# luo-yining/CFDBench

Hardware: NVIDIA H100
Metric: fno_rollout_steps_per_sec (higher is better)
Workload: dtype bf16

## Files before the change

cfdbench_b200/_lib.py:

```python
from __future__ import annotations

import ctypes as C
import os

_HERE = os.path.dirname(os.path.abspath(__file__))
LIB_PATH = os.path.join(_HERE, "libcfdbench_b200.so")

FNO_MAX_LAYERS = 8
ABI_VERSION = 4
ACT_F32, ACT_BF16 = 0, 1
EPI_GELU, EPI_GELU_SAVE_PRE, EPI_MUL_DGELU, EPI_PLAIN = 0, 1, 2, 3


class FnoWeights(C.Structure):
    _fields_ = [
        ("n_layers", C.c_int32),
        ("n_case_params", C.c_int32),
        ("fc0_w", C.c_void_p),
        ("fc0_b", C.c_void_p),
        ("spec_wk", C.c_void_p * FNO_MAX_LAYERS),
        ("w0t", C.c_void_p * FNO_MAX_LAYERS),
        ("w0_b", C.c_void_p * FNO_MAX_LAYERS),
        ("fc1_w", C.c_void_p),
        ("fc1_b", C.c_void_p),
# ... 64 lines not shown
    "fno_bwd_partials_bytes": (C.c_size_t, []),
    "fno_mode_mix_image": (C.c_int, [_P, _P, _P, _I, _P]),
    "fno_block_fused": (C.c_int, [_P, _P, _P, _P, _P, _I, _P]),
    "fno_pack_spectral_weights": (C.c_int, [_P, _P, _P, _I, _P]),
    "fno_unpack_spectral_grads": (C.c_int, [_P, _P, _P, _P]),
    "fno_mix_operand_bytes": (C.c_size_t, []),
    "fno_pack_mix_operand": (C.c_int, [_P, _P, _P]),
    "fno_pack_mix_operand_from_weights": (C.c_int, [_P, _P, _P, _I, _P]),
    "fno_lift_fwd": (C.c_int, [_P, _P, _P, C.POINTER(FnoWeights), _P, _I, _I, _P]),
    "fno_spectral_dft_fwd": (C.c_int, [_P, _P, _I, _I, _F, _F, _P]),
    "fno_mode_mix": (C.c_int, [_P, _P, _P, _I, _P]),
    "fno_spectral_inv_kx": (C.c_int, [_P, _P, _I, _F, _F, _P]),
    "fno_block_out": (C.c_int, [_I, _P, _P, _P, _P, _P, _P, _P, _I, _I, _P]),
    "fno_block_fwd": (C.c_int, [C.POINTER(FnoWeights), _I, _P, _P, _P, C.POINTER(FnoWorkspace), _I, _I, _P]),
    "fno_project_fwd": (C.c_int, [_P, _P, C.POINTER(FnoWeights), _P, _I, _I, _P]),
    "fno_forward": (C.c_int, [C.POINTER(FnoWeights), _P, _P, _P, _P, C.POINTER(FnoWorkspace), _I, _I, _P]),
    "fno_rollout": (C.c_int, [C.POINTER(FnoWeights), _P, _P, _P, _P, _I, C.POINTER(FnoWorkspace), _I, _I, _P]),
    "fno_rollout_host": (C.c_int, [C.POINTER(FnoWeights), _P, _P, _P, _P, _I, C.POINTER(FnoWorkspace), _P, _I, _I, _P]),
    "fno_rollout_host_scratch_bytes": (C.c_size_t, [_I, _I, _I]),
    "fno_multistep_metrics": (C.c_int, [_P, _P, _P, _P, _I, _I, _P]),
    "fno_gather_batch": (C.c_int, [_P, _P, _P, _P, _P, _I, _I, _I, _P, _P, _P, _P, _P]),
    "fno_loss_scratch_bytes": (C.c_size_t, []),
    "fno_loss_fwd": (C.c_int, [_P, _P, C.c_size_t, _P, _P, _P]),
    "fno_loss_bwd": (C.c_int, [_P, _P, _P, _P, _P, C.c_size_t, _P]),
    "fno_adam_step": (C.c_int, [C.POINTER(FnoAdamTensors), C.c_float, C.c_float, C.c_float, C.c_float, C.c_float,
                                C.c_int64, _P]),
    "fno_train_stage_indices": (C.c_int, [_P, C.c_int64, _I, _I, _P, _P, _P]),
    "fno_adam_step_dev": (C.c_int, [C.POINTER(FnoAdamTensors), _P, _I, _P, _F, _F, _F, _F, _P]),
    "fno_adam_coefficients": (C.c_int, [_F, _F, _F, C.c_int64, _I, _P]),
    "fno_train_log_step": (C.c_int, [_P, _P, _I, _P, _P]),
# ... 78 lines not shown
```

cfdbench_b200/build.py:

```python
from __future__ import annotations

import hashlib
import os
import subprocess
import sys
import time

HERE = os.path.dirname(os.path.abspath(__file__))
CSRC = os.path.join(HERE, "csrc")
OUT = os.path.join(HERE, "libcfdbench_b200.so")
STAMP = os.path.join(HERE, ".build_stamp")
SOURCES = ["fno_abi.cu", "fno_dft_fwd.cu", "fno_dft_fwd_tc.cu", "fno_mode_mix.cu", "fno_block_tc.cu", "fno_block_fused.cu", "fno_pointwise.cu", "fno_project_tc.cu", "fno_project_bwd_tc.cu",
           "fno_backward.cu", "fno_metrics.cu", "fno_train_step.cu", "fno_grid.cu"]
NVCC_FLAGS = ["-std=c++17", "-O3", "-lineinfo", "-gencode", "arch=compute_90a,code=sm_90a",
              "-Xcompiler", "-fPIC"]


def _nvcc() -> str:
    for cand in (os.environ.get("NVCC"), "/usr/local/cuda/bin/nvcc"):
        if cand and os.path.exists(cand):
            return cand
    return "nvcc"


def _fingerprint() -> str:
    h = hashlib.sha256()
    for root in (CSRC, os.path.join(os.path.dirname(HERE), "include")):
# ... 52 lines not shown
```

cfdbench_b200/csrc/fno_abi.cu:

```cuda
#include <stdio.h>
#include <string.h>

#include "../../include/cfdbench_b200.h"
#include "fno_common.cuh"

namespace fno {
cudaError_t launch_dft_fwd(const void*, void*, int, float, float, cudaStream_t);
cudaError_t launch_mode_mix(const void*, const void*, void*, void*, int, cudaStream_t);
cudaError_t launch_block_fused(const void*, const void*, const float*, const float*, void*, int, cudaStream_t);
size_t ym_image_bytes(int);
cudaError_t launch_pack_spectral(const void*, const void*, void*, int, cudaStream_t);
cudaError_t launch_unpack_spectral(const void*, void*, void*, int, cudaStream_t);
cudaError_t launch_dft_fwd_tc(const void*, void*, int, float, float, cudaStream_t);
cudaError_t launch_pack_mix_operand(const void*, void*, cudaStream_t);
cudaError_t launch_pack_mix_operand_direct(const void*, const void*, void*, int, cudaStream_t);
size_t mix_operand_bytes();
cudaError_t launch_gather_batch(const void*, const void*, const float*, const int*, const long long*, int, int, int, float*,
                                float*, float*, float*, cudaStream_t);
cudaError_t launch_loss_fwd(const float*, const float*, size_t, float*, float*, cudaStream_t);
cudaError_t launch_loss_bwd(const float*, const float*, const float*, const float*, float*, size_t, cudaStream_t);
size_t loss_scratch_bytes();
cudaError_t launch_adam_step(const fno_adam_tensors*, float, float, float, float, float, long long, cudaStream_t);
cudaError_t launch_adam_step_dev(const fno_adam_tensors*, const float*, int, const int*, float, float, float, float,
                                 cudaStream_t);
void adam_coefficients(float, float, float, long long, float*, float*);
cudaError_t launch_stage_indices(const long long*, long long, int, int, const int*, long long*, cudaStream_t);
cudaError_t launch_log_step(const float*, float*, int, int*, cudaStream_t);
cudaError_t launch_inv_kx(const void*, void*, int, float, float, cudaStream_t);
template <typename TAct>
cudaError_t launch_block_tc(int, const void*, const void*, const float*, const float*, void*, float*, const float*, int,
                            cudaStream_t);
template <typename TAct>
cudaError_t launch_lift(const float*, const float*, const float*, const float*, const float*, const float*,
                        const float*, void*, int, int, cudaStream_t);
template <typename TAct>
cudaError_t launch_project_tc(const void*, const float*, const float*, const float*, const float*, const float*,
                              float*, int, cudaStream_t);
int project_bwd_rows_max();
int project_bwd_row();
cudaError_t launch_reduce_partials(const float*, int, int, float*, int, float*, int, float*, int, int, cudaStream_t);
template <typename TAct>
cudaError_t launch_project_bwd_tc(const void*, const float*, const float*, const float*, const float*, const float*, const float*,
                                  float*, float*, float*, int*, int, cudaStream_t);
template <typename TP, typename TQ, int NJ, int NI>
cudaError_t launch_chan_outer(const void*, const void*, float*, int*, int, cudaStream_t);
cudaError_t launch_multistep_metrics(const float*, const float*, const float*, float*, int, int, cudaStream_t);
cudaError_t launch_spectral_wgrad(const void*, const void*, void*, int, cudaStream_t);
cudaError_t launch_lift_bwd(const float*, const float*, const float*, const float*, const float*, const float*,
                            float*, float*, float*, int, int, int, cudaStream_t);
cudaError_t launch_lift_bwd_data(const float*, const float*, float*, float*, const float*, int, int, int, cudaStream_t);
bool grid_ok(int, int);
void grid_tables_release(int);
// ... 186 lines not shown
  if (act_dtype == FNO_ACT_BF16 && ws->ym_img && !pre_out) {
    FNO_TRY(fno_mode_mix_image(ws->xm, w->spec_wk[layer], ws->ym_img, batch, stream));
    return fno_block_fused(ws->ym_img, act_in, w->w0t[layer], w->w0_b[layer], act_out, batch, stream);
  }
  FNO_TRY(fno_mode_mix(ws->xm, w->spec_wk[layer], ws->ym, batch, stream));
  const float inv = 1.f / static_cast<float>(kHW);
  FNO_TRY(fno_spectral_inv_kx(ws->ym, ws->z, batch, inv, 2.f * inv, stream));
  return fno_block_out(pre_out ? FNO_EPI_GELU_SAVE_PRE : FNO_EPI_GELU, ws->z, act_in, w->w0t[layer], w->w0_b[layer],
                       act_out, pre_out, nullptr, batch, act_dtype, stream);
}

int fno_project_fwd(const void* act_in, const float* mask, const fno_weights* w, float* preds, int batch,
                    int act_dtype, void* stream) {
  if (!act_in || !mask || !w || !preds || batch <= 0 || bad_dtype(act_dtype))
    return fail(kErrArg, "fno_project_fwd: bad argument");
  cudaError_t e =
      act_dtype == FNO_ACT_F32
          ? launch_project_tc<float>(act_in, w->fc1_w, w->fc1_b, w->fc2_w, w->fc2_b, mask, preds, batch, S(stream))
          : launch_project_tc<__nv_bfloat16>(act_in, w->fc1_w, w->fc1_b, w->fc2_w, w->fc2_b, mask, preds, batch, S(stream));
  FNO_CUDA(e, "project_kernel");
  return kOk;
}

int fno_forward(const fno_weights* w, const float* inputs, const float* mask, const float* case_params,
                float* preds, const fno_workspace* ws, int batch, int act_dtype, void* stream) {
  if (!w || !ws || !ws->act[0] || !ws->act[1] || !ws->xm) return fail(kErrArg, "fno_forward: bad workspace");
  if (!(act_dtype == FNO_ACT_BF16 && ws->ym_img) && (!ws->ym || !ws->z)) return fail(kErrArg, "fno_forward: bad workspace");
  if (w->n_layers < 1 || w->n_layers > FNO_MAX_LAYERS) return fail(kErrUnsupported, "fno_forward: n_layers out of range");
  FNO_TRY(fno_lift_fwd(inputs, mask, case_params, w, ws->act[0], batch, act_dtype, stream));
  int cur = 0;
  for (int l = 0; l < w->n_layers; ++l) {
    FNO_TRY(fno_block_fwd(w, l, ws->act[cur], ws->act[cur ^ 1], nullptr, ws, batch, act_dtype, stream));
    cur ^= 1;
  }
  return fno_project_fwd(ws->act[cur], mask, w, preds, batch, act_dtype, stream);
}

int fno_rollout(const fno_weights* w, const float* inputs, const float* mask, const float* case_params,
                float* preds_seq, int steps, const fno_workspace* ws, int batch, int act_dtype, void* stream) {
  if (steps < 0 || !preds_seq) return fail(kErrArg, "fno_rollout: bad argument");
  const size_t frame = static_cast<size_t>(batch) * 2 * kHW;
  const float* cur = inputs;
  for (int s = 0; s < steps; ++s) {
    float* nxt = preds_seq + static_cast<size_t>(s) * frame;
    FNO_TRY(fno_forward(w, cur, mask, case_params, nxt, ws, batch, act_dtype, stream));
    cur = nxt;
  }
  return kOk;
}

size_t fno_rollout_host_scratch_bytes(int batch, int n_case_params, int steps) {
  const size_t b = static_cast<size_t>(batch);
  return (b * 2 * kHW + b * kHW + static_cast<size_t>(steps) * b * 2 * kHW) * sizeof(float) +
         ((b * n_case_params * sizeof(float) + 255) / 256) * 256;
}

int fno_rollout_host(const fno_weights* w, const float* inputs_host, const float* mask_host,
                     const float* case_params_host, float* preds_seq_host, int steps, const fno_workspace* ws,
                     void* dev_io, int batch, int act_dtype, void* stream) {
  if (!w || !inputs_host || !mask_host || !preds_seq_host || !dev_io || batch <= 0 || steps <= 0)
    return fail(kErrArg, "fno_rollout_host: bad argument");
// ... 677 lines not shown
```

cfdbench_b200/csrc/fno_project_tc.cu:

```cuda
#include "fno_common.cuh"
#include "tc_common.cuh"

namespace fno {

constexpr int kPtWG = 4;
constexpr int kPtThreads = 128 * kPtWG;
constexpr int kPtM = kW;
constexpr uint32_t kPtLboA = (kPtM / 8) * 128;
constexpr uint32_t kPtLboB = (kProj / 8) * 128;
constexpr int kPtTilesPerSample = kH;
constexpr int kPtReps = kPtM * (kC / 4) / 128;

struct PtSmem {
  alignas(128) float w_hi[kProj * kC];
  alignas(128) float w_lo[kProj * kC];
  alignas(128) float a_hi[kPtWG][kPtM * kC];
  alignas(128) float a_lo[kPtWG][kPtM * kC];
  alignas(16) float4 w2q[kProj / 2];
  alignas(16) float2 b1p[kProj / 2];
};

template <typename TAct>
struct PtRegs {
  TAct v[kPtReps][4];
};

template <typename TAct>
__device__ __forceinline__ void pt_prefetch(PtRegs<TAct>& r, const TAct* __restrict__ a, int tile, int t) {
  const int b = tile / kPtTilesPerSample, p0 = (tile % kPtTilesPerSample) * kPtM;
#pragma unroll
  for (int rep = 0; rep < kPtReps; ++rep) {
    const int task = rep * 128 + t;
    const int m = task & (kPtM - 1), kq = task >> 6;
    const TAct* src = a + (static_cast<size_t>(b) * kC + 4 * kq) * kHW + p0 + m;
#pragma unroll
    for (int c = 0; c < 4; ++c) r.v[rep][c] = __ldg(src + static_cast<size_t>(c) * kHW);
  }
}

__device__ __forceinline__ float pt_to_float(float v) { return v; }
__device__ __forceinline__ float pt_to_float(__nv_bfloat16 v) { return __bfloat162float(v); }

template <typename TAct>
__device__ __forceinline__ void pt_split_store(const PtRegs<TAct>& r, float* a_hi, float* a_lo, int t) {
#pragma unroll
  for (int rep = 0; rep < kPtReps; ++rep) {
    const int task = rep * 128 + t;
    const int m = task & (kPtM - 1), kq = task >> 6;
    float hi[4], lo[4];
#pragma unroll
    for (int c = 0; c < 4; ++c) {
      const float x = pt_to_float(r.v[rep][c]);
      if constexpr (sizeof(TAct) == 4) tc::split_tf32(x, hi[c], lo[c]);
      else hi[c] = x;
    }
    const uint32_t off = tc::kmajor_offset(m, 4 * kq, kPtM) / 4;
    *reinterpret_cast<float4*>(a_hi + off) = make_float4(hi[0], hi[1], hi[2], hi[3]);
    if constexpr (sizeof(TAct) == 4) *reinterpret_cast<float4*>(a_lo + off) = make_float4(lo[0], lo[1], lo[2], lo[3]);
  }
}

template <typename TAct>
__global__ void __launch_bounds__(kPtThreads, 1)
    project_tc_kernel(const TAct* __restrict__ a, const float* __restrict__ w1, const float* __restrict__ b1,
                      const float* __restrict__ w2, const float* __restrict__ b2, const float* __restrict__ mask,
                      float* __restrict__ preds, int n_tiles) {
  constexpr bool kBf16 = sizeof(TAct) == 2;
  extern __shared__ __align__(1024) unsigned char smem_raw[];
  PtSmem& sm = *reinterpret_cast<PtSmem*>(smem_raw);
  const int tid = threadIdx.x, lane = tid & 31;
  const int wg = tc::warp_index_uniform() >> 2, t = tid & 127, wq = (tid >> 5) & 3;

  for (int e = tid; e < kProj * kC; e += kPtThreads) {
    const int j = e / kC, i = e % kC;
    float hi, lo;
    tc::split_tf32(w1[e], hi, lo);
    const uint32_t off = tc::kmajor_offset(j, i, kProj) / 4;
    sm.w_hi[off] = hi;
    sm.w_lo[off] = lo;
  }
  if (tid < kProj / 2) {
    sm.w2q[tid] = make_float4(w2[2 * tid], w2[kProj + 2 * tid], w2[2 * tid + 1], w2[kProj + 2 * tid + 1]);
    sm.b1p[tid] = make_float2(b1[2 * tid], b1[2 * tid + 1]);
  }
  const float b2x = b2[0], b2y = b2[1];
  tc::fence_proxy_async_smem();
  __syncthreads();
  pdl_wait();
  pdl_launch_dependents();

  const int first = blockIdx.x * kPtWG + wg, stride = gridDim.x * kPtWG;
  float* a_hi = sm.a_hi[wg];
  float* a_lo = sm.a_lo[wg];
  PtRegs<TAct> regs;
  if (first < n_tiles) pt_prefetch<TAct>(regs, a, first, t);
  for (int tile = first; tile < n_tiles; tile += stride) {
    pt_split_store<TAct>(regs, a_hi, a_lo, t);
    tc::fence_proxy_async_smem();
    tc::named_barrier(1 + wg, 128);
    if (tile + stride < n_tiles) pt_prefetch<TAct>(regs, a, tile + stride, t);
    float acc[64];
    tc::wg_fence();
    {
      const uint32_t a_s[3] = {tc::smem_addr(a_hi), tc::smem_addr(a_lo), tc::smem_addr(a_hi)};
      const uint32_t b_s[3] = {tc::smem_addr(sm.w_hi), tc::smem_addr(sm.w_hi), tc::smem_addr(sm.w_lo)};
#pragma unroll
      for (int pass = 0; pass < 3; ++pass) {
        if (kBf16 && pass == 1) continue;
#pragma unroll
        for (int ks = 0; ks < kC / 8; ++ks)
          tc::wg_tf32_ss_n128(acc, tc::make_smem_desc(a_s[pass] + ks * 2 * kPtLboA, kPtLboA, 128),
                              tc::make_smem_desc(b_s[pass] + ks * 2 * kPtLboB, kPtLboB, 128), (pass | ks) ? 1u : 0u);
      }
    }
    tc::wg_commit();
    tc::wg_wait<0>();
    tc::wg_fence_acc(acc);
    const int b = tile / kPtTilesPerSample, p0 = (tile % kPtTilesPerSample) * kPtM;
#pragma unroll
    for (int hh = 0; hh < 2; ++hh) {
      float2 out = make_float2(0.f, 0.f);
#pragma unroll
      for (int i0 = 0; i0 < 16; i0 += 8) {
        float2 g[8];
#pragma unroll
        for (int i = 0; i < 8; ++i) {
          const float2 bb = sm.b1p[4 * (i0 + i) + (lane & 3)];
          g[i] = make_float2(acc[4 * (i0 + i) + 2 * hh] + bb.x, acc[4 * (i0 + i) + 2 * hh + 1] + bb.y);
        }
        if constexpr (kBf16) {
          gelu_erf2_deg5_batch<8>(g);
        } else {
#pragma unroll
          for (int i = 0; i < 8; ++i) g[i] = gelu_erf2(g[i]);
        }
#pragma unroll
        for (int i = 0; i < 8; ++i) {
          const float4 wq4 = sm.w2q[4 * (i0 + i) + (lane & 3)];
          out = ffma2(make_float2(g[i].x, g[i].x), make_float2(wq4.x, wq4.y), out);
          out = ffma2(make_float2(g[i].y, g[i].y), make_float2(wq4.z, wq4.w), out);
        }
      }
      out.x += __shfl_xor_sync(0xffffffffu, out.x, 1);
      out.y += __shfl_xor_sync(0xffffffffu, out.y, 1);
      out.x += __shfl_xor_sync(0xffffffffu, out.x, 2);
      out.y += __shfl_xor_sync(0xffffffffu, out.y, 2);
      if ((lane & 3) == 0) {
        const int pix = p0 + 16 * wq + (lane >> 2) + 8 * hh;
        const float mk = __ldg(mask + static_cast<size_t>(b) * kHW + pix);
        preds[(static_cast<size_t>(b) * 2 + 0) * kHW + pix] = (b2x + out.x) * mk;
        preds[(static_cast<size_t>(b) * 2 + 1) * kHW + pix] = (b2y + out.y) * mk;
      }
    }
  }
}

template <typename TAct>
cudaError_t launch_project_tc(const void* a, const float* w1, const float* b1, const float* w2, const float* b2,
                              const float* mask, float* preds, int batch, cudaStream_t stream) {
  auto kern = project_tc_kernel<TAct>;
  constexpr size_t smem = sizeof(PtSmem);
  static PerDeviceLaunch pd;
  int n_sm = 0;
  cudaError_t e0 = per_device_setup(kern, smem, pd, &n_sm);
  if (e0 != cudaSuccess) return e0;
  const int n_tiles = batch * kPtTilesPerSample;
  const int want = (n_tiles + kPtWG - 1) / kPtWG;
  const int grid = want < n_sm ? want : n_sm;
  return launch_chained(kern, dim3(grid), dim3(kPtThreads), smem, stream, static_cast<const TAct*>(a), w1, b1, w2, b2,
                        mask, preds, n_tiles);
}
template cudaError_t launch_project_tc<float>(const void*, const float*, const float*, const float*, const float*,
                                              const float*, float*, int, cudaStream_t);
template cudaError_t launch_project_tc<__nv_bfloat16>(const void*, const float*, const float*, const float*,
                                                      const float*, const float*, float*, int, cudaStream_t);

}
```

cfdbench_b200/csrc/tc_common.cuh:

```cuda
#pragma once
#include <cuda_runtime.h>
#include <stdint.h>

namespace fno {
namespace tc {

__device__ __forceinline__ uint32_t smem_addr(const void* p) {
  return static_cast<uint32_t>(__cvta_generic_to_shared(p));
}

__device__ __forceinline__ int warp_index_uniform() {
  return __shfl_sync(0xffffffffu, static_cast<int>(threadIdx.x >> 5), 0);
}

__device__ __forceinline__ void named_barrier(int id, int count) {
  asm volatile("bar.sync %0, %1;" ::"r"(id), "r"(count) : "memory");
}

__device__ __forceinline__ void fence_proxy_async_smem() {
  asm volatile("fence.proxy.async.shared::cta;" ::: "memory");
}

__device__ __forceinline__ uint64_t make_smem_desc(uint32_t saddr, uint32_t lbo_bytes, uint32_t sbo_bytes) {
  uint64_t d = 0;
// ... 39 lines not shown
  asm volatile(
      "{\n.reg .pred p;\nsetp.ne.b32 p, %38, 0;\n"
      "wgmma.mma_async.sync.aligned.m64n72k16.f32.bf16.bf16 {%0, %1, %2, %3, %4, %5, %6, %7, %8, %9, %10, %11, %12, %13, %14, %15, %16, %17, %18, %19, %20, %21, %22, %23, %24, %25, %26, %27, %28, %29, %30, %31, %32, %33, %34, %35}, %36, %37, p, 1, 1, 0, 0;\n}\n"
      : "+f"(d[0]), "+f"(d[1]), "+f"(d[2]), "+f"(d[3]), "+f"(d[4]), "+f"(d[5]), "+f"(d[6]), "+f"(d[7]), "+f"(d[8]), "+f"(d[9]), "+f"(d[10]), "+f"(d[11]), "+f"(d[12]), "+f"(d[13]), "+f"(d[14]), "+f"(d[15]), "+f"(d[16]), "+f"(d[17]), "+f"(d[18]), "+f"(d[19]), "+f"(d[20]), "+f"(d[21]), "+f"(d[22]), "+f"(d[23]), "+f"(d[24]), "+f"(d[25]), "+f"(d[26]), "+f"(d[27]), "+f"(d[28]), "+f"(d[29]), "+f"(d[30]), "+f"(d[31]), "+f"(d[32]), "+f"(d[33]), "+f"(d[34]), "+f"(d[35])
      : "l"(a), "l"(b), "r"(acc)
      : "memory");
}
__device__ __forceinline__ void wg_bf16_ss_n32_mn_a(float* d, uint64_t a, uint64_t b, uint32_t acc) {
  asm volatile(
      "{\n.reg .pred p;\nsetp.ne.b32 p, %18, 0;\n"
      "wgmma.mma_async.sync.aligned.m64n32k16.f32.bf16.bf16 {%0, %1, %2, %3, %4, %5, %6, %7, %8, %9, %10, %11, %12, %13, %14, %15}, %16, %17, p, 1, 1, 1, 0;\n}\n"
      : "+f"(d[0]), "+f"(d[1]), "+f"(d[2]), "+f"(d[3]), "+f"(d[4]), "+f"(d[5]), "+f"(d[6]), "+f"(d[7]), "+f"(d[8]), "+f"(d[9]), "+f"(d[10]), "+f"(d[11]), "+f"(d[12]), "+f"(d[13]), "+f"(d[14]), "+f"(d[15])
      : "l"(a), "l"(b), "r"(acc)
      : "memory");
}
__device__ __forceinline__ void wg_tf32_rs_n32(float* d, const uint32_t* a, uint64_t b, uint32_t acc) {
  asm volatile(
      "{\n.reg .pred p;\nsetp.ne.b32 p, %21, 0;\n"
      "wgmma.mma_async.sync.aligned.m64n32k8.f32.tf32.tf32 {%0, %1, %2, %3, %4, %5, %6, %7, %8, %9, %10, %11, %12, %13, %14, %15}, {%16, %17, %18, %19}, %20, p, 1, 1;\n}\n"
      : "+f"(d[0]), "+f"(d[1]), "+f"(d[2]), "+f"(d[3]), "+f"(d[4]), "+f"(d[5]), "+f"(d[6]), "+f"(d[7]), "+f"(d[8]), "+f"(d[9]), "+f"(d[10]), "+f"(d[11]), "+f"(d[12]), "+f"(d[13]), "+f"(d[14]), "+f"(d[15])
      : "r"(a[0]), "r"(a[1]), "r"(a[2]), "r"(a[3]), "l"(b), "r"(acc)
      : "memory");
}
__device__ __forceinline__ void wg_tf32_rs_n48(float* d, const uint32_t* a, uint64_t b, uint32_t acc) {
  asm volatile(
      "{\n.reg .pred p;\nsetp.ne.b32 p, %29, 0;\n"
      "wgmma.mma_async.sync.aligned.m64n48k8.f32.tf32.tf32 {%0, %1, %2, %3, %4, %5, %6, %7, %8, %9, %10, %11, %12, %13, %14, %15, %16, %17, %18, %19, %20, %21, %22, %23}, {%24, %25, %26, %27}, %28, p, 1, 1;\n}\n"
      : "+f"(d[0]), "+f"(d[1]), "+f"(d[2]), "+f"(d[3]), "+f"(d[4]), "+f"(d[5]), "+f"(d[6]), "+f"(d[7]), "+f"(d[8]), "+f"(d[9]), "+f"(d[10]), "+f"(d[11]), "+f"(d[12]), "+f"(d[13]), "+f"(d[14]), "+f"(d[15]), "+f"(d[16]), "+f"(d[17]), "+f"(d[18]), "+f"(d[19]), "+f"(d[20]), "+f"(d[21]), "+f"(d[22]), "+f"(d[23])
      : "r"(a[0]), "r"(a[1]), "r"(a[2]), "r"(a[3]), "l"(b), "r"(acc)
      : "memory");
// ... 24 lines not shown
```

include/cfdbench_b200.h:

```cpp
#ifndef CFDBENCH_B200_H_
#define CFDBENCH_B200_H_

#include <stddef.h>
#include <stdint.h>

#ifdef __cplusplus
extern "C" {
#endif

#define FNO_ABI_VERSION 4
#define FNO_MAX_LAYERS 8

enum { FNO_ACT_F32 = 0, FNO_ACT_BF16 = 1 };
enum { FNO_EPI_GELU = 0, FNO_EPI_GELU_SAVE_PRE = 1, FNO_EPI_MUL_DGELU = 2, FNO_EPI_PLAIN = 3 };

typedef struct fno_weights {
  int32_t n_layers;
  int32_t n_case_params;
  const float* fc0_w;
  const float* fc0_b;
  const void* spec_wk[FNO_MAX_LAYERS];
  const float* w0t[FNO_MAX_LAYERS];
  const float* w0_b[FNO_MAX_LAYERS];
  const float* fc1_w;
// ... 32 lines not shown
                 void* act_out, int batch, int act_dtype, void* stream);

int fno_spectral_dft_fwd(const void* act_in, void* xm, int batch, int act_dtype, float s0, float s1, void* stream);
int fno_mode_mix(const void* xm, const void* wop, void* ym, int batch, void* stream);
int fno_spectral_inv_kx(const void* ym, void* z, int batch, float s0, float s1, void* stream);
int fno_block_out(int epilogue, const void* z, const void* act_in, const float* w0t, const float* bias, void* act_out,
                  float* pre_out, const float* pre_in, int batch, int act_dtype, void* stream);
int fno_mode_mix_image(const void* xm, const void* wop, void* ym_img, int batch, void* stream);
int fno_block_fused(const void* ym_img, const void* act_in_bf16, const float* w0t, const float* bias, void* act_out_bf16,
                    int batch, void* stream);
int fno_block_fwd(const fno_weights* w, int layer, const void* act_in, void* act_out, float* pre_out,
                  const fno_workspace* ws, int batch, int act_dtype, void* stream);

int fno_project_fwd(const void* act_in, const float* mask, const fno_weights* w, float* preds, int batch,
                    int act_dtype, void* stream);

int fno_forward(const fno_weights* w, const float* inputs, const float* mask, const float* case_params,
                float* preds, const fno_workspace* ws, int batch, int act_dtype, void* stream);

int fno_rollout(const fno_weights* w, const float* inputs, const float* mask, const float* case_params,
                float* preds_seq, int steps, const fno_workspace* ws, int batch, int act_dtype, void* stream);

int fno_rollout_host(const fno_weights* w, const float* inputs_host, const float* mask_host,
                     const float* case_params_host, float* preds_seq_host, int steps, const fno_workspace* ws,
                     void* dev_io, int batch, int act_dtype, void* stream);
size_t fno_rollout_host_scratch_bytes(int batch, int n_case_params, int steps);


typedef struct fno_train_saved {
  void* act[FNO_MAX_LAYERS + 1];
// ... 149 lines not shown
```

Before: 1258.

## Fuse bf16 projection with next-step lift in rollout using TMA-fed wgmma kernel

```diff
diff --git a/cfdbench_b200/_lib.py b/cfdbench_b200/_lib.py
--- a/cfdbench_b200/_lib.py
+++ b/cfdbench_b200/_lib.py
@@ -102,6 +102,7 @@
     "fno_block_out": (C.c_int, [_I, _P, _P, _P, _P, _P, _P, _P, _I, _I, _P]),
     "fno_block_fwd": (C.c_int, [C.POINTER(FnoWeights), _I, _P, _P, _P, C.POINTER(FnoWorkspace), _I, _I, _P]),
     "fno_project_fwd": (C.c_int, [_P, _P, C.POINTER(FnoWeights), _P, _I, _I, _P]),
+    "fno_project_lift_fwd": (C.c_int, [_P, _P, _P, C.POINTER(FnoWeights), _P, _P, _I, _P]),
     "fno_forward": (C.c_int, [C.POINTER(FnoWeights), _P, _P, _P, _P, C.POINTER(FnoWorkspace), _I, _I, _P]),
     "fno_rollout": (C.c_int, [C.POINTER(FnoWeights), _P, _P, _P, _P, _I, C.POINTER(FnoWorkspace), _I, _I, _P]),
     "fno_rollout_host": (C.c_int, [C.POINTER(FnoWeights), _P, _P, _P, _P, _I, C.POINTER(FnoWorkspace), _P, _I, _I, _P]),
diff --git a/cfdbench_b200/build.py b/cfdbench_b200/build.py
--- a/cfdbench_b200/build.py
+++ b/cfdbench_b200/build.py
@@ -10,7 +10,7 @@
 CSRC = os.path.join(HERE, "csrc")
 OUT = os.path.join(HERE, "libcfdbench_b200.so")
 STAMP = os.path.join(HERE, ".build_stamp")
-SOURCES = ["fno_abi.cu", "fno_dft_fwd.cu", "fno_dft_fwd_tc.cu", "fno_mode_mix.cu", "fno_block_tc.cu", "fno_block_fused.cu", "fno_pointwise.cu", "fno_project_tc.cu", "fno_project_bwd_tc.cu",
+SOURCES = ["fno_abi.cu", "fno_dft_fwd.cu", "fno_dft_fwd_tc.cu", "fno_mode_mix.cu", "fno_block_tc.cu", "fno_block_fused.cu", "fno_pointwise.cu", "fno_project_tc.cu", "fno_project_bf16.cu", "fno_project_bwd_tc.cu",
            "fno_backward.cu", "fno_metrics.cu", "fno_train_step.cu", "fno_grid.cu"]
 NVCC_FLAGS = ["-std=c++17", "-O3", "-lineinfo", "-gencode", "arch=compute_90a,code=sm_90a",
               "-Xcompiler", "-fPIC"]
diff --git a/cfdbench_b200/csrc/fno_abi.cu b/cfdbench_b200/csrc/fno_abi.cu
--- a/cfdbench_b200/csrc/fno_abi.cu
+++ b/cfdbench_b200/csrc/fno_abi.cu
@@ -33,9 +33,12 @@
 template <typename TAct>
 cudaError_t launch_lift(const float*, const float*, const float*, const float*, const float*, const float*,
                         const float*, void*, int, int, cudaStream_t);
-template <typename TAct>
 cudaError_t launch_project_tc(const void*, const float*, const float*, const float*, const float*, const float*,
                               float*, int, cudaStream_t);
+template <bool kLift>
+cudaError_t launch_project_bf16(const void*, const float*, const float*, const float*, const float*, const float*, float*,
+                                const float*, const float*, const float*, const float*, const float*, int, void*, int,
+                                cudaStream_t);
 int project_bwd_rows_max();
 int project_bwd_row();
 cudaError_t launch_reduce_partials(const float*, int, int, float*, int, float*, int, float*, int, int, cudaStream_t);
@@ -252,25 +255,60 @@
                     int act_dtype, void* stream) {
   if (!act_in || !mask || !w || !preds || batch <= 0 || bad_dtype(act_dtype))
     return fail(kErrArg, "fno_project_fwd: bad argument");
-  cudaError_t e =
-      act_dtype == FNO_ACT_F32
-          ? launch_project_tc<float>(act_in, w->fc1_w, w->fc1_b, w->fc2_w, w->fc2_b, mask, preds, batch, S(stream))
-          : launch_project_tc<__nv_bfloat16>(act_in, w->fc1_w, w->fc1_b, w->fc2_w, w->fc2_b, mask, preds, batch, S(stream));
-  FNO_CUDA(e, "project_kernel");
+  if (act_dtype == FNO_ACT_BF16) {
+    FNO_CUDA(launch_project_bf16<false>(act_in, w->fc1_w, w->fc1_b, w->fc2_w, w->fc2_b, mask, preds, nullptr, nullptr,
+                                        nullptr, nullptr, nullptr, 0, nullptr, batch, S(stream)),
+             "project_bf16_kernel");
+    return kOk;
+  }
+  FNO_CUDA(launch_project_tc(act_in, w->fc1_w, w->fc1_b, w->fc2_w, w->fc2_b, mask, preds, batch, S(stream)),
+           "project_tc_kernel");
+  return kOk;
+}
+
+int fno_project_lift_fwd(const void* act_in, const float* mask, const float* case_params, const fno_weights* w,
+                         float* preds, void* act_next, int batch, void* stream) {
+  if (!act_in || !mask || !w || !preds || !act_next || batch <= 0 || act_in == act_next || !w->gx || !w->gy)
+    return fail(kErrArg, "fno_project_lift_fwd: bad argument");
+  if (w->n_case_params < 0 || w->n_case_params > kMaxCaseParams)
+    return fail(kErrUnsupported, "fno_project_lift_fwd: n_case_params out of range");
+  if (w->n_case_params > 0 && !case_params) return fail(kErrArg, "fno_project_lift_fwd: case_params is null");
+  if ((reinterpret_cast<uintptr_t>(act_in) | reinterpret_cast<uintptr_t>(act_next)) & 15)
+    return fail(kErrArg, "fno_project_lift_fwd: act_in and act_next must be 16-byte aligned");
+  FNO_CUDA(launch_project_bf16<true>(act_in, w->fc1_w, w->fc1_b, w->fc2_w, w->fc2_b, mask, preds, w->fc0_w, w->fc0_b,
+                                     case_params, w->gx, w->gy, w->n_case_params, act_next, batch, S(stream)),
+           "project_bf16_kernel<lift>");
+  return kOk;
+}
+
+static int forward_ws_args(const char* what, const fno_weights* w, const fno_workspace* ws, int act_dtype) {
+  char msg[128];
+  if (!w || !ws || !ws->act[0] || !ws->act[1] || !ws->xm ||
+      (!(act_dtype == FNO_ACT_BF16 && ws->ym_img) && (!ws->ym || !ws->z))) {
+    snprintf(msg, sizeof(msg), "%s: bad workspace", what);
+    return fail(kErrArg, msg);
+  }
+  if (w->n_layers < 1 || w->n_layers > FNO_MAX_LAYERS) {
+    snprintf(msg, sizeof(msg), "%s: n_layers out of range", what);
+    return fail(kErrUnsupported, msg);
+  }
+  return kOk;
+}
+
+static int forward_layers(const fno_weights* w, const fno_workspace* ws, int* cur, int batch, int act_dtype, void* stream) {
+  for (int l = 0; l < w->n_layers; ++l) {
+    FNO_TRY(fno_block_fwd(w, l, ws->act[*cur], ws->act[*cur ^ 1], nullptr, ws, batch, act_dtype, stream));
+    *cur ^= 1;
+  }
   return kOk;
 }
 
 int fno_forward(const fno_weights* w, const float* inputs, const float* mask, const float* case_params,
                 float* preds, const fno_workspace* ws, int batch, int act_dtype, void* stream) {
-  if (!w || !ws || !ws->act[0] || !ws->act[1] || !ws->xm) return fail(kErrArg, "fno_forward: bad workspace");
-  if (!(act_dtype == FNO_ACT_BF16 && ws->ym_img) && (!ws->ym || !ws->z)) return fail(kErrArg, "fno_forward: bad workspace");
-  if (w->n_layers < 1 || w->n_layers > FNO_MAX_LAYERS) return fail(kErrUnsupported, "fno_forward: n_layers out of range");
+  FNO_TRY(forward_ws_args("fno_forward", w, ws, act_dtype));
   FNO_TRY(fno_lift_fwd(inputs, mask, case_params, w, ws->act[0], batch, act_dtype, stream));
   int cur = 0;
-  for (int l = 0; l < w->n_layers; ++l) {
-    FNO_TRY(fno_block_fwd(w, l, ws->act[cur], ws->act[cur ^ 1], nullptr, ws, batch, act_dtype, stream));
-    cur ^= 1;
-  }
+  FNO_TRY(forward_layers(w, ws, &cur, batch, act_dtype, stream));
   return fno_project_fwd(ws->act[cur], mask, w, preds, batch, act_dtype, stream);
 }
 
@@ -278,11 +316,25 @@
                 float* preds_seq, int steps, const fno_workspace* ws, int batch, int act_dtype, void* stream) {
   if (steps < 0 || !preds_seq) return fail(kErrArg, "fno_rollout: bad argument");
   const size_t frame = static_cast<size_t>(batch) * 2 * kHW;
-  const float* cur = inputs;
+  if (act_dtype != FNO_ACT_BF16) {
+    const float* cur = inputs;
+    for (int s = 0; s < steps; ++s) {
+      float* nxt = preds_seq + static_cast<size_t>(s) * frame;
+      FNO_TRY(fno_forward(w, cur, mask, case_params, nxt, ws, batch, act_dtype, stream));
+      cur = nxt;
+    }
+    return kOk;
+  }
+  if (steps == 0) return kOk;
+  FNO_TRY(forward_ws_args("fno_rollout", w, ws, act_dtype));
+  FNO_TRY(fno_lift_fwd(inputs, mask, case_params, w, ws->act[0], batch, act_dtype, stream));
+  int cur = 0;
   for (int s = 0; s < steps; ++s) {
     float* nxt = preds_seq + static_cast<size_t>(s) * frame;
-    FNO_TRY(fno_forward(w, cur, mask, case_params, nxt, ws, batch, act_dtype, stream));
-    cur = nxt;
+    FNO_TRY(forward_layers(w, ws, &cur, batch, act_dtype, stream));
+    if (s == steps - 1) return fno_project_fwd(ws->act[cur], mask, w, nxt, batch, act_dtype, stream);
+    FNO_TRY(fno_project_lift_fwd(ws->act[cur], mask, case_params, w, nxt, ws->act[cur ^ 1], batch, stream));
+    cur ^= 1;
   }
   return kOk;
 }
diff --git a/cfdbench_b200/csrc/fno_project_bf16.cu b/cfdbench_b200/csrc/fno_project_bf16.cu
--- /dev/null
+++ b/cfdbench_b200/csrc/fno_project_bf16.cu
@@ -0,0 +1,261 @@
+#include "fno_common.cuh"
+#include "tc_common.cuh"
+#include "tc_tma.cuh"
+
+namespace fno {
+
+constexpr int kPbWG = 4;
+constexpr int kPbThreads = 128 * kPbWG;
+constexpr uint32_t kPbBoxW = kW, kPbBoxH = 1, kPbBoxC = kC;
+constexpr uint32_t kPbRowBytes = kPbBoxW * kPbBoxH * kPbBoxC * 2;
+constexpr int kPbXSlots = 4;
+constexpr uint32_t kPbW1Bytes = kProj * kC * 2;
+constexpr uint32_t kPbLboW1 = (kProj / 8) * 128;
+constexpr int kPbChains = 4;
+constexpr uint32_t kPbHalfBytes = (kProj / 2 / 8) * 128;
+
+__host__ __device__ constexpr int pb_tile_begin(int gp, int n_pipes, int n_tiles) {
+  return static_cast<int>(static_cast<long long>(gp) * n_tiles / n_pipes);
+}
+__host__ __device__ constexpr int pb_x_slot(int n) { return n % kPbXSlots; }
+__host__ __device__ constexpr uint32_t pb_x_parity(int n) { return static_cast<uint32_t>(n / kPbXSlots) & 1u; }
+
+struct PbSmem {
+  alignas(1024) unsigned char x[kPbWG][kPbXSlots][kPbRowBytes];
+  alignas(1024) unsigned char st[kPbWG][2][kPbRowBytes];
+  alignas(128) unsigned char w1[3][kPbW1Bytes];
+  alignas(16) float4 w2q[kProj / 2];
+  alignas(16) float2 b1p[kProj / 2];
+  alignas(16) float4 lw[kC];
+  float lwp[kC][kMaxCaseParams + 2];
+  float lbase[kPbWG][2][kC];
+  float gy[kW];
+  alignas(8) uint64_t x_full[kPbWG][kPbXSlots];
+};
+static_assert(sizeof(PbSmem) <= 232448, "project_bf16_kernel: shared memory over the per-block opt-in limit");
+
+__device__ __forceinline__ void pb_issue_half(float (&d)[32], uint32_t a_x, uint32_t w1_half) {
+  tc::wg_fence();
+#pragma unroll
+  for (int term = 0; term < 3; ++term)
+#pragma unroll
+    for (int ks = 0; ks < kC / 16; ++ks)
+      tc::wg_bf16_ss_n64_mn_a(d, tc::make_smem_desc_sw128_mn(a_x + ks * 2048),
+                              tc::make_smem_desc(w1_half + term * kPbW1Bytes + ks * 2 * kPbLboW1, kPbLboW1, 128),
+                              (term | ks) ? 1u : 0u);
+  tc::wg_commit();
+}
+
+__device__ __forceinline__ void pb_epilogue_half(const float (&d)[32], const PbSmem& sm, int half, int q, float2 (&out)[2]) {
+#pragma unroll
+  for (int hh = 0; hh < 2; ++hh)
+#pragma unroll
+    for (int i0 = 0; i0 < 8; i0 += kPbChains) {
+      float2 g[kPbChains];
+#pragma unroll
+      for (int i = 0; i < kPbChains; ++i) {
+        const float2 bb = sm.b1p[4 * (8 * half + i0 + i) + q];
+        g[i] = make_float2(__fadd_rn(d[4 * (i0 + i) + 2 * hh], bb.x), __fadd_rn(d[4 * (i0 + i) + 2 * hh + 1], bb.y));
+      }
+      gelu_erf2_deg5_batch<kPbChains>(g);
+#pragma unroll
+      for (int i = 0; i < kPbChains; ++i) {
+        const float4 wq4 = sm.w2q[4 * (8 * half + i0 + i) + q];
+        out[hh] = ffma2(make_float2(g[i].x, g[i].x), make_float2(wq4.x, wq4.y), out[hh]);
+        out[hh] = ffma2(make_float2(g[i].y, g[i].y), make_float2(wq4.z, wq4.w), out[hh]);
+      }
+    }
+}
+
+__device__ __forceinline__ uint32_t pb_sw128_offset(int line, int e) {
+  return static_cast<uint32_t>(line * 128 + ((((e >> 3) ^ line) & 7) << 4) + (e & 7) * 2);
+}
+
+template <bool kLift>
+__global__ void __launch_bounds__(kPbThreads, 1)
+    project_bf16_kernel(const __grid_constant__ CUtensorMap x_map, const __grid_constant__ CUtensorMap out_map,
+                        const float* __restrict__ w1, const float* __restrict__ b1, const float* __restrict__ w2,
+                        const float* __restrict__ b2, const float* __restrict__ mask, float* __restrict__ preds,
+                        const float* __restrict__ lift_w, const float* __restrict__ lift_b,
+                        const float* __restrict__ params, const float* __restrict__ gx, const float* __restrict__ gy,
+                        int p, int n_tiles) {
+  extern __shared__ __align__(1024) unsigned char smem_raw[];
+  PbSmem& sm = *reinterpret_cast<PbSmem*>(smem_raw);
+  if ((smem_u32(smem_raw) & 1023u) != 0) __trap();
+  const int tid = threadIdx.x, lane = tid & 31;
+  const int wg = tc::warp_index_uniform() >> 2, t = tid & 127, wq = (tid >> 5) & 3, q = lane & 3;
+
+  if (tid == 0) {
+    for (int g = 0; g < kPbWG; ++g)
+      for (int s = 0; s < kPbXSlots; ++s) mbar_init(&sm.x_full[g][s], 1);
+    fence_mbar_init();
+  }
+  for (int e = tid; e < kProj * kC; e += kPbThreads) {
+    const int j = e / kC, i = e % kC;
+    const float w = w1[e];
+    const __nv_bfloat16 t1 = __float2bfloat16_rn(w);
+    const float r1 = w - __bfloat162float(t1);
+    const __nv_bfloat16 t2 = __float2bfloat16_rn(r1);
+    const __nv_bfloat16 t3 = __float2bfloat16_rn(r1 - __bfloat162float(t2));
+    const uint32_t off = static_cast<uint32_t>(((i >> 3) * (kProj / 8) + (j >> 3)) * 128 + (j & 7) * 16 + (i & 7) * 2);
+    *reinterpret_cast<__nv_bfloat16*>(sm.w1[0] + off) = t1;
+    *reinterpret_cast<__nv_bfloat16*>(sm.w1[1] + off) = t2;
+    *reinterpret_cast<__nv_bfloat16*>(sm.w1[2] + off) = t3;
+  }
+  if (tid < kProj / 2) {
+    sm.w2q[tid] = make_float4(w2[2 * tid], w2[kProj + 2 * tid], w2[2 * tid + 1], w2[kProj + 2 * tid + 1]);
+    sm.b1p[tid] = make_float2(b1[2 * tid], b1[2 * tid + 1]);
+  }
+  if constexpr (kLift) {
+    const int nin = 5 + p;
+    if (tid < kC) {
+      sm.lw[tid] = make_float4(lift_w[tid * nin + 0], lift_w[tid * nin + 1], lift_w[tid * nin + 2], lift_w[tid * nin + 4]);
+      for (int qq = 0; qq < p; ++qq) sm.lwp[tid][qq] = lift_w[tid * nin + 5 + qq];
+      sm.lwp[tid][kMaxCaseParams] = lift_w[tid * nin + 3];
+      sm.lwp[tid][kMaxCaseParams + 1] = lift_b[tid];
+    }
+    if (tid < kW) sm.gy[tid] = gy[tid];
+  }
+  const float b2x = b2[0], b2y = b2[1];
+  tc::fence_proxy_async_smem();
+  __syncthreads();
+  pdl_wait();
+  pdl_launch_dependents();
+
+  const int n_pipes = gridDim.x * kPbWG, gp = blockIdx.x * kPbWG + wg;
+  const int tile0 = pb_tile_begin(gp, n_pipes, n_tiles), n_own = pb_tile_begin(gp + 1, n_pipes, n_tiles) - tile0;
+  auto x_fill = [&](int n) {
+    const int tile = tile0 + n, s = pb_x_slot(n);
+    mbar_expect_tx(&sm.x_full[wg][s], kPbRowBytes);
+    tma_load_3d(sm.x[wg][s], &x_map, 0, tile % kH, (tile / kH) * kC, &sm.x_full[wg][s]);
+  };
+  if (t == 0)
+    for (int n = 0; n < kPbXSlots && n < n_own; ++n) x_fill(n);
+  const uint32_t w1_s = tc::smem_addr(sm.w1[0]);
+  auto lift_base = [&](int n) {
+    if (t < kC) {
+      const int tile = tile0 + n, b = tile / kH, c = t;
+      float cb = sm.lwp[c][kMaxCaseParams + 1];
+      for (int qq = 0; qq < p; ++qq) cb = fmaf(sm.lwp[c][qq], params[b * p + qq], cb);
+      sm.lbase[wg][n & 1][c] = fmaf(sm.lwp[c][kMaxCaseParams], gx[tile % kH], cb);
+    }
+  };
+
+  float acc0[32], acc1[32];
+  auto tile_step = [&](int n, bool more) {
+    const int tile = tile0 + n, b = tile / kH, h = tile % kH;
+    float2 out[2] = {make_float2(0.f, 0.f), make_float2(0.f, 0.f)};
+    tc::wg_wait<1>();
+    tc::wg_fence_acc(acc0);
+    pb_epilogue_half(acc0, sm, 0, q, out);
+    if (more) {
+      const int s1 = pb_x_slot(n + 1);
+      mbar_wait(&sm.x_full[wg][s1], pb_x_parity(n + 1));
+      pb_issue_half(acc0, tc::smem_addr(sm.x[wg][s1]), w1_s);
+      tc::wg_wait<1>();
+    } else {
+      tc::wg_wait<0>();
+    }
+    tc::wg_fence_acc(acc1);
+    pb_epilogue_half(acc1, sm, 1, q, out);
+
+    const float* mrow = mask + static_cast<size_t>(b) * kHW + h * kW;
+    float* prow = preds + static_cast<size_t>(b) * 2 * kHW + h * kW;
+    unsigned char* stile = sm.st[wg][n & 1];
+    float u[2], v[2], mk[2];
+#pragma unroll
+    for (int hh = 0; hh < 2; ++hh) {
+      float2 o = out[hh];
+      o.x = __fadd_rn(o.x, __shfl_xor_sync(0xffffffffu, o.x, 1));
+      o.y = __fadd_rn(o.y, __shfl_xor_sync(0xffffffffu, o.y, 1));
+      o.x = __fadd_rn(o.x, __shfl_xor_sync(0xffffffffu, o.x, 2));
+      o.y = __fadd_rn(o.y, __shfl_xor_sync(0xffffffffu, o.y, 2));
+      const int px = 16 * wq + (lane >> 2) + 8 * hh;
+      mk[hh] = __ldg(mrow + px);
+      u[hh] = __fmul_rn(__fadd_rn(b2x, o.x), mk[hh]);
+      v[hh] = __fmul_rn(__fadd_rn(b2y, o.y), mk[hh]);
+      if (q == 0) prow[px] = u[hh];
+      if (q == 1) prow[kHW + px] = v[hh];
+    }
+    if constexpr (kLift) {
+      const float* lbase = sm.lbase[wg][n & 1];
+      const int px0 = 16 * wq + (lane >> 2);
+      const float yw[2] = {sm.gy[px0], sm.gy[px0 + 8]};
+#pragma unroll
+      for (int j = 0; j < kC / 4; ++j) {
+        const int c = 4 * j + q;
+        const float4 lw = sm.lw[c];
+        const float base = lbase[c];
+#pragma unroll
+        for (int hh = 0; hh < 2; ++hh) {
+          const float r = fmaf(lw.x, u[hh], fmaf(lw.y, v[hh], fmaf(lw.z, mk[hh], fmaf(lw.w, yw[hh], base))));
+          *reinterpret_cast<__nv_bfloat16*>(stile + pb_sw128_offset(c, px0 + 8 * hh)) = __float2bfloat16_rn(r);
+        }
+      }
+    }
+    if (more) pb_issue_half(acc1, tc::smem_addr(sm.x[wg][pb_x_slot(n + 1)]), w1_s + kPbHalfBytes);
+    if constexpr (kLift) {
+      if (more) lift_base(n + 1);
+      tc::fence_proxy_async_smem();
+      if (t == 0) bulk_wait_group_read<0>();
+    }
+    tc::named_barrier(1 + wg, 128);
+    if (t == 0) {
+      if constexpr (kLift) {
+        tma_store_3d(&out_map, stile, 0, h, b * kC);
+        bulk_commit_group();
+      }
+      if (n + kPbXSlots < n_own) x_fill(n + kPbXSlots);
+    }
+  };
+  if (n_own > 0) {
+    if constexpr (kLift) {
+      lift_base(0);
+      tc::named_barrier(1 + wg, 128);
+    }
+    mbar_wait(&sm.x_full[wg][pb_x_slot(0)], pb_x_parity(0));
+    pb_issue_half(acc0, tc::smem_addr(sm.x[wg][pb_x_slot(0)]), w1_s);
+    pb_issue_half(acc1, tc::smem_addr(sm.x[wg][pb_x_slot(0)]), w1_s + kPbHalfBytes);
+    for (int n = 0; n + 1 < n_own; ++n) tile_step(n, true);
+    tile_step(n_own - 1, false);
+  }
+  if constexpr (kLift) {
+    if (t == 0) bulk_wait_group<0>();
+  }
+}
+
+template <bool kLift>
+cudaError_t launch_project_bf16(const void* a, const float* w1, const float* b1, const float* w2, const float* b2,
+                                const float* mask, float* preds, const float* lift_w, const float* lift_b,
+                                const float* params, const float* gx, const float* gy, int p, void* a_next, int batch,
+                                cudaStream_t stream) {
+  auto kern = project_bf16_kernel<kLift>;
+  static PerDeviceLaunch pd;
+  int n_sm = 0;
+  cudaError_t e = per_device_setup(kern, sizeof(PbSmem), pd, &n_sm);
+  if (e != cudaSuccess) return e;
+  if ((reinterpret_cast<uintptr_t>(a) & 15) || (reinterpret_cast<uintptr_t>(a_next) & 15))
+    return cudaErrorMisalignedAddress;
+  CUtensorMap x_map, out_map;
+  const uint64_t planes = static_cast<uint64_t>(batch) * kC;
+  e = make_tma_map_3d(&x_map, CU_TENSOR_MAP_DATA_TYPE_BFLOAT16, 2, a, kW, kH, planes, kPbBoxW, kPbBoxH, kPbBoxC);
+  if (e != cudaSuccess) return e;
+  out_map = x_map;
+  if (kLift) {
+    e = make_tma_map_3d(&out_map, CU_TENSOR_MAP_DATA_TYPE_BFLOAT16, 2, a_next, kW, kH, planes, kPbBoxW, kPbBoxH, kPbBoxC);
+    if (e != cudaSuccess) return e;
+  }
+  const int n_tiles = batch * kH;
+  const int want = (n_tiles + kPbWG - 1) / kPbWG;
+  const int grid = want < n_sm ? want : n_sm;
+  return launch_chained(kern, dim3(grid), dim3(kPbThreads), sizeof(PbSmem), stream, x_map, out_map, w1, b1, w2, b2, mask,
+                        preds, lift_w, lift_b, params, gx, gy, p, n_tiles);
+}
+template cudaError_t launch_project_bf16<false>(const void*, const float*, const float*, const float*, const float*,
+                                                const float*, float*, const float*, const float*, const float*,
+                                                const float*, const float*, int, void*, int, cudaStream_t);
+template cudaError_t launch_project_bf16<true>(const void*, const float*, const float*, const float*, const float*,
+                                               const float*, float*, const float*, const float*, const float*,
+                                               const float*, const float*, int, void*, int, cudaStream_t);
+
+}
diff --git a/cfdbench_b200/csrc/fno_project_tc.cu b/cfdbench_b200/csrc/fno_project_tc.cu
--- a/cfdbench_b200/csrc/fno_project_tc.cu
+++ b/cfdbench_b200/csrc/fno_project_tc.cu
@@ -20,52 +20,40 @@
   alignas(16) float2 b1p[kProj / 2];
 };
 
-template <typename TAct>
 struct PtRegs {
-  TAct v[kPtReps][4];
+  float v[kPtReps][4];
 };
 
-template <typename TAct>
-__device__ __forceinline__ void pt_prefetch(PtRegs<TAct>& r, const TAct* __restrict__ a, int tile, int t) {
+__device__ __forceinline__ void pt_prefetch(PtRegs& r, const float* __restrict__ a, int tile, int t) {
   const int b = tile / kPtTilesPerSample, p0 = (tile % kPtTilesPerSample) * kPtM;
 #pragma unroll
   for (int rep = 0; rep < kPtReps; ++rep) {
     const int task = rep * 128 + t;
     const int m = task & (kPtM - 1), kq = task >> 6;
-    const TAct* src = a + (static_cast<size_t>(b) * kC + 4 * kq) * kHW + p0 + m;
+    const float* src = a + (static_cast<size_t>(b) * kC + 4 * kq) * kHW + p0 + m;
 #pragma unroll
     for (int c = 0; c < 4; ++c) r.v[rep][c] = __ldg(src + static_cast<size_t>(c) * kHW);
   }
 }
 
-__device__ __forceinline__ float pt_to_float(float v) { return v; }
-__device__ __forceinline__ float pt_to_float(__nv_bfloat16 v) { return __bfloat162float(v); }
-
-template <typename TAct>
-__device__ __forceinline__ void pt_split_store(const PtRegs<TAct>& r, float* a_hi, float* a_lo, int t) {
+__device__ __forceinline__ void pt_split_store(const PtRegs& r, float* a_hi, float* a_lo, int t) {
 #pragma unroll
   for (int rep = 0; rep < kPtReps; ++rep) {
     const int task = rep * 128 + t;
     const int m = task & (kPtM - 1), kq = task >> 6;
     float hi[4], lo[4];
 #pragma unroll
-    for (int c = 0; c < 4; ++c) {
-      const float x = pt_to_float(r.v[rep][c]);
-      if constexpr (sizeof(TAct) == 4) tc::split_tf32(x, hi[c], lo[c]);
-      else hi[c] = x;
-    }
+    for (int c = 0; c < 4; ++c) tc::split_tf32(r.v[rep][c], hi[c], lo[c]);
     const uint32_t off = tc::kmajor_offset(m, 4 * kq, kPtM) / 4;
     *reinterpret_cast<float4*>(a_hi + off) = make_float4(hi[0], hi[1], hi[2], hi[3]);
-    if constexpr (sizeof(TAct) == 4) *reinterpret_cast<float4*>(a_lo + off) = make_float4(lo[0], lo[1], lo[2], lo[3]);
+    *reinterpret_cast<float4*>(a_lo + off) = make_float4(lo[0], lo[1], lo[2], lo[3]);
   }
 }
 
-template <typename TAct>
 __global__ void __launch_bounds__(kPtThreads, 1)
-    project_tc_kernel(const TAct* __restrict__ a, const float* __restrict__ w1, const float* __restrict__ b1,
+    project_tc_kernel(const float* __restrict__ a, const float* __restrict__ w1, const float* __restrict__ b1,
                       const float* __restrict__ w2, const float* __restrict__ b2, const float* __restrict__ mask,
                       float* __restrict__ preds, int n_tiles) {
-  constexpr bool kBf16 = sizeof(TAct) == 2;
   extern __shared__ __align__(1024) unsigned char smem_raw[];
   PtSmem& sm = *reinterpret_cast<PtSmem*>(smem_raw);
   const int tid = threadIdx.x, lane = tid & 31;
@@ -92,13 +80,13 @@
   const int first = blockIdx.x * kPtWG + wg, stride = gridDim.x * kPtWG;
   float* a_hi = sm.a_hi[wg];
   float* a_lo = sm.a_lo[wg];
-  PtRegs<TAct> regs;
-  if (first < n_tiles) pt_prefetch<TAct>(regs, a, first, t);
+  PtRegs regs;
+  if (first < n_tiles) pt_prefetch(regs, a, first, t);
   for (int tile = first; tile < n_tiles; tile += stride) {
-    pt_split_store<TAct>(regs, a_hi, a_lo, t);
+    pt_split_store(regs, a_hi, a_lo, t);
     tc::fence_proxy_async_smem();
     tc::named_barrier(1 + wg, 128);
-    if (tile + stride < n_tiles) pt_prefetch<TAct>(regs, a, tile + stride, t);
+    if (tile + stride < n_tiles) pt_prefetch(regs, a, tile + stride, t);
     float acc[64];
     tc::wg_fence();
     {
@@ -106,7 +94,6 @@
       const uint32_t b_s[3] = {tc::smem_addr(sm.w_hi), tc::smem_addr(sm.w_hi), tc::smem_addr(sm.w_lo)};
 #pragma unroll
       for (int pass = 0; pass < 3; ++pass) {
-        if (kBf16 && pass == 1) continue;
 #pragma unroll
         for (int ks = 0; ks < kC / 8; ++ks)
           tc::wg_tf32_ss_n128(acc, tc::make_smem_desc(a_s[pass] + ks * 2 * kPtLboA, kPtLboA, 128),
@@ -128,12 +115,8 @@
           const float2 bb = sm.b1p[4 * (i0 + i) + (lane & 3)];
           g[i] = make_float2(acc[4 * (i0 + i) + 2 * hh] + bb.x, acc[4 * (i0 + i) + 2 * hh + 1] + bb.y);
         }
-        if constexpr (kBf16) {
-          gelu_erf2_deg5_batch<8>(g);
-        } else {
 #pragma unroll
-          for (int i = 0; i < 8; ++i) g[i] = gelu_erf2(g[i]);
-        }
+        for (int i = 0; i < 8; ++i) g[i] = gelu_erf2(g[i]);
 #pragma unroll
         for (int i = 0; i < 8; ++i) {
           const float4 wq4 = sm.w2q[4 * (i0 + i) + (lane & 3)];
@@ -155,10 +138,9 @@
   }
 }
 
-template <typename TAct>
 cudaError_t launch_project_tc(const void* a, const float* w1, const float* b1, const float* w2, const float* b2,
                               const float* mask, float* preds, int batch, cudaStream_t stream) {
-  auto kern = project_tc_kernel<TAct>;
+  auto kern = project_tc_kernel;
   constexpr size_t smem = sizeof(PtSmem);
   static PerDeviceLaunch pd;
   int n_sm = 0;
@@ -167,12 +149,8 @@
   const int n_tiles = batch * kPtTilesPerSample;
   const int want = (n_tiles + kPtWG - 1) / kPtWG;
   const int grid = want < n_sm ? want : n_sm;
-  return launch_chained(kern, dim3(grid), dim3(kPtThreads), smem, stream, static_cast<const TAct*>(a), w1, b1, w2, b2,
+  return launch_chained(kern, dim3(grid), dim3(kPtThreads), smem, stream, static_cast<const float*>(a), w1, b1, w2, b2,
                         mask, preds, n_tiles);
 }
-template cudaError_t launch_project_tc<float>(const void*, const float*, const float*, const float*, const float*,
-                                              const float*, float*, int, cudaStream_t);
-template cudaError_t launch_project_tc<__nv_bfloat16>(const void*, const float*, const float*, const float*,
-                                                      const float*, const float*, float*, int, cudaStream_t);
 
 }
diff --git a/cfdbench_b200/csrc/tc_common.cuh b/cfdbench_b200/csrc/tc_common.cuh
--- a/cfdbench_b200/csrc/tc_common.cuh
+++ b/cfdbench_b200/csrc/tc_common.cuh
@@ -77,6 +77,14 @@
       : "l"(a), "l"(b), "r"(acc)
       : "memory");
 }
+__device__ __forceinline__ void wg_bf16_ss_n64_mn_a(float* d, uint64_t a, uint64_t b, uint32_t acc) {
+  asm volatile(
+      "{\n.reg .pred p;\nsetp.ne.b32 p, %34, 0;\n"
+      "wgmma.mma_async.sync.aligned.m64n64k16.f32.bf16.bf16 {%0, %1, %2, %3, %4, %5, %6, %7, %8, %9, %10, %11, %12, %13, %14, %15, %16, %17, %18, %19, %20, %21, %22, %23, %24, %25, %26, %27, %28, %29, %30, %31}, %32, %33, p, 1, 1, 1, 0;\n}\n"
+      : "+f"(d[0]), "+f"(d[1]), "+f"(d[2]), "+f"(d[3]), "+f"(d[4]), "+f"(d[5]), "+f"(d[6]), "+f"(d[7]), "+f"(d[8]), "+f"(d[9]), "+f"(d[10]), "+f"(d[11]), "+f"(d[12]), "+f"(d[13]), "+f"(d[14]), "+f"(d[15]), "+f"(d[16]), "+f"(d[17]), "+f"(d[18]), "+f"(d[19]), "+f"(d[20]), "+f"(d[21]), "+f"(d[22]), "+f"(d[23]), "+f"(d[24]), "+f"(d[25]), "+f"(d[26]), "+f"(d[27]), "+f"(d[28]), "+f"(d[29]), "+f"(d[30]), "+f"(d[31])
+      : "l"(a), "l"(b), "r"(acc)
+      : "memory");
+}
 __device__ __forceinline__ void wg_tf32_rs_n32(float* d, const uint32_t* a, uint64_t b, uint32_t acc) {
   asm volatile(
       "{\n.reg .pred p;\nsetp.ne.b32 p, %21, 0;\n"
diff --git a/include/cfdbench_b200.h b/include/cfdbench_b200.h
--- a/include/cfdbench_b200.h
+++ b/include/cfdbench_b200.h
@@ -70,6 +70,8 @@
 
 int fno_project_fwd(const void* act_in, const float* mask, const fno_weights* w, float* preds, int batch,
                     int act_dtype, void* stream);
+int fno_project_lift_fwd(const void* act_in, const float* mask, const float* case_params, const fno_weights* w,
+                         float* preds, void* act_next, int batch, void* stream);
 
 int fno_forward(const fno_weights* w, const float* inputs, const float* mask, const float* case_params,
                 float* preds, const fno_workspace* ws, int batch, int act_dtype, void* stream);
```

Result: no change. 1272, median of 6 (+1.1%).
